# ru1ven/KeypointFusion

Hardware: AMD Instinct MI355X
Metric: RGB-D img/sec fwd (B=64, 256x256) (higher is better)
Workload: dtype f32; 1 GPU; KPFusion-convnext-tiny, depth+RGB UNet backbones forward, B=64/GPU 256x256 f32 (BASELINE configs[1]); batch_per_gpu=64, global_batch=64, input=256x256, parallelism=dp1 (batch shards, no collective)

## Files before the change

include/kpf.h:

```cpp
#ifndef KPF_H
#define KPF_H

#ifdef __cplusplus
extern "C" {
#endif

#define KPF_OK 0
#define KPF_EINVAL (-1)
#define KPF_ELAUNCH (-2)

#define KPF_DT_F32 0
#define KPF_DT_BF16 1
#define KPF_DT_F16 2
#define KPF_DT_F32_MMA_BF16 8
#define KPF_DT_F32_MMA_F16 9

#define KPF_ACT_RELU 1u
#define KPF_ACT_GELU 2u
#define KPF_RES_ADD 4u
#define KPF_RES_GAMMA 8u
#define KPF_RELU_AFTER_RES 16u
#define KPF_ACT_LEAKY 64u
#define KPF_IN_SPLIT 128u
#define KPF_W_SPLIT 512u
#define KPF_OUT_SPLIT 256u
#define KPF_OUT_NCHW 32u
#define KPF_ACT_GELU_SAVE 2048u
#define KPF_MMA_BF16 8192u
#define KPF_MMA_F16 16384u
#define KPF_PRO_LN 4096u
#define KPF_RES_GELU_GRAD 1024u

typedef struct kpf_conv_desc {
  int B, IH, IW, Cin;
  int in_ld, in_coff;
  int OH, OW, N;
  int KH, KW, sh, sw, ph, pw;
  int Kp;
  int out_ld, out_coff;
  int res_ld, res_coff;
  unsigned flags;
  float w_unscale;
  int tile_cfg;
  int groups;
  long w_gstride;
} kpf_conv_desc;

int kpf_conv2d_f32(const kpf_conv_desc* d, const float* in, const float* w, const float* bias,
                   const float* pro_scale, const float* pro_shift, const float* gamma, const float* res,
                   float* out, void* stream);

int kpf_dwconv7_ln_f32(const float* x, const float* w_dw, const float* b_dw, const float* ln_w, const float* ln_b,
                       float* y, int B, int H, int W, int C, float eps, void* stream);

int kpf_convnext_mlp_f32(const float* y, const float* x, const float* w1, const float* b1, const float* w2, const float* b2,
                         const float* gamma, float* out, long M, int C, void* stream);
int kpf_convnext_mlp_supported(int C);
int kpf_convnext_mlp_split_f32(const float* y_split, const float* x, const float* w1_split, const float* b1, float w1_unscale,
                               const float* w2_split_perm, const float* b2, float w2_unscale, const float* gamma, float* out, long M,
                               int C, void* stream);
int kpf_convnext_mlp_split_supported(int C);
int kpf_convnext_mlp_h16(const void* y, const void* x, const void* w1, const float* b1, const void* w2_chunks, const float* b2,
                         const float* gamma, void* out, long M, int C, int dtype, void* stream);
int kpf_convnext_mlp_h16_supported(int C);

int kpf_dwconv7_stats_h16(const void* x, const float* w_dw, const float* b_dw, void* y, float* stats, int B, int H, int W, int C, int dtype,
                          void* stream);
int kpf_dwconv7_stats_supported(int H, int W, int C);
long kpf_dwconv7_stats_floats(int B, int H, int W, int C);
int kpf_ln_apply_stats_h16(void* y, const float* stats, const float* ln_w, const float* ln_b, long rows, int C, float eps, int dtype, void* stream);
int kpf_ln_stats_merge(const float* stats, float* mean_rstd, long rows, int C, float eps, void* stream);

int kpf_layernorm_f32(const float* x, const float* w, const float* b, float* y, long rows, int C, float eps, void* stream);

int kpf_dwconv7_ln_split_f32(const float* x, const float* w_dw, const float* b_dw, const float* ln_w, const float* ln_b, float* y,
                             int B, int H, int W, int C, float eps, void* stream);
int kpf_layernorm_split_f32(const float* x, const float* w, const float* b, float* y, long rows, int C, float eps, void* stream);

int kpf_upsample2x_f32(const float* src, float* dst, int B, int H, int W, int C, int dst_ld, int dst_coff, void* stream);

int kpf_nchw_to_nhwc_f32(const float* src, float* dst, int B, int C, int H, int W, int Cpad, void* stream);

int kpf_nhwc_to_nchw_f32(const float* src, float* dst, int B, int C, int H, int W, int src_ld, int src_coff, void* stream);
// ... 321 lines not shown
```

keypointfusion_amd/csrc/kpf_conv.hip:

```cpp
#include "kpf_common.h"
#include <stdlib.h>
#include <type_traits>

namespace {

struct ConvArgs {
  const float* in;
  const float* w;
  const float* bias;
  const float* ps;
  const float* pt;
  const float* gamma;
  const float* res;
  float* out;
  int M, N, K, Kp;
  int IH, IW, Cin, in_ld, in_coff;
  int OH, OW, ohow, KH, KW, sh, sw, ph, pw;
  int out_ld, out_coff, res_ld, res_coff;
  const float* zero;
  float w_unscale;
  unsigned flags;
  int tilesN, nblk;
  int vec;
  int dbg;
// ... 29 lines not shown
__device__ __forceinline__ float gelu_h16(float x) { return kpf_gelu_h16(x); }
enum { ARITH_F32 = 0, ARITH_SPLIT = 1, ARITH_SPLIT_W = 2, ARITH_BF16 = 3, ARITH_F16 = 4, ARITH_R_BF16 = 5, ARITH_R_F16 = 6 };
template <int ARITH>
__device__ __forceinline__ float gelu_of(float x) {
  if constexpr (ARITH == ARITH_BF16 || ARITH == ARITH_F16) return gelu_h16(x);
  else return gelu_erf(x);
}

enum { EPI_LIN = 0, EPI_GELU = 1, EPI_RES = 2, EPI_GGRAD = 3, EPI_GELU2 = 4 };
__device__ __forceinline__ float gelu_exact_erf(float v) { return 0.5f * v * (1.0f + erff(v * 0.70710678118654752440f)); }
__device__ __forceinline__ float gelu_grad_erf(float v) {
  const float cdf = 0.5f * (1.0f + erff(v * 0.70710678118654752440f));
  return cdf + v * 0.3989422804014327f * __expf(-0.5f * v * v);
}
#ifndef STORE4
#define STORE4(p, v) *reinterpret_cast<f32x4*>(p) = (v)
#endif

typedef __attribute__((address_space(3))) void lds_void_t;
typedef __attribute__((address_space(1))) void gbl_void_t;

__device__ __attribute__((aligned(16))) float kpf_zero16[4] = {0.f, 0.f, 0.f, 0.f};

#ifdef KPF_DBG_TIME
__device__ unsigned long long kpf_dbg_t[8 * 8192];
#define KPF_STAMP(i) do { if (threadIdx.x == 0 && blockIdx.x < 8192) { kpf_dbg_t[8 * blockIdx.x + (i)] = __builtin_readcyclecounter(); \
    if ((i) == 0) { kpf_dbg_t[8 * blockIdx.x + 4] = __builtin_amdgcn_s_memrealtime(); kpf_dbg_t[8 * blockIdx.x + 6] = __builtin_amdgcn_s_getreg((4 << 0) | (0 << 6) | (31 << 11)) | ((unsigned long long)__builtin_amdgcn_s_getreg((20 << 0) | (0 << 6) | (3 << 11)) << 32); } \
    if ((i) == 3) kpf_dbg_t[8 * blockIdx.x + 5] = __builtin_amdgcn_s_memrealtime(); } } while (0)
#else
#define KPF_STAMP(i)
#endif
constexpr int BK = 32;

template <int TM, int TN, int WM, int WN, bool IS1X1, bool HAS_PRO, int EPI, int ARITH, int NS>
__device__ __forceinline__ void igemm_body(const ConvArgs& a) {
  constexpr bool SPLIT = ARITH == ARITH_SPLIT || ARITH == ARITH_SPLIT_W;
  constexpr bool H16 = ARITH == ARITH_BF16 || ARITH == ARITH_F16;
  using TH = typename std::conditional<ARITH == ARITH_BF16, bf16_t, f16_t>::type;
  constexpr int BM = 16 * TM * WM;
  constexpr int BN = 16 * TN * WN;
  constexpr int NW = WM * WN;
  constexpr int RPP = 8 * NW;
  constexpr int AP = (BM + RPP - 1) / RPP;
  constexpr int BP = (BN + RPP - 1) / RPP;
  constexpr bool R16 = ARITH == ARITH_R_BF16 || ARITH == ARITH_R_F16;
  constexpr bool WHOLE = NS > 2 || ARITH == ARITH_F32 || R16;
  constexpr int BMR = WHOLE ? AP * RPP : BM;
  constexpr int BNR = WHOLE ? BP * RPP : BN;
  constexpr int TILE = (BMR + BNR) * BK;
  constexpr int CNT = AP + BP;
  static_assert(NW == 4 || NW == 8, "4 or 8 waves per workgroup");
  static_assert(NS >= 1 && (NS < 2 || (NS - 2) * CNT < 64), "vmcnt is a 6-bit counter");
  static_assert(BM % 8 == 0 && BN % 8 == 0, "tile granularity");

  extern __shared__ __attribute__((aligned(16))) float lds[];

  const int tid = threadIdx.x;
  const int lane = tid & 63;
  const int wave = __builtin_amdgcn_readfirstlane(tid >> 6);
  const int wm = wave % WM, wn = wave / WM;
  KPF_STAMP(0);
  if constexpr (ARITH == ARITH_F32 && NS == 2) {
    if (a.skew > 0 && (int)blockIdx.x < 512 && blockIdx.y == 0) {
      const unsigned tg = __builtin_amdgcn_s_getreg(4 | (16 << 6) | (3 << 11));
      if (tg & 1)
        for (int i = 0; i < a.skew; ++i) __builtin_amdgcn_s_sleep(32);
    }
  }
// ... 111 lines not shown
    }
  }
  if (NS <= 2) __syncthreads();

  KPF_STAMP(1);
  if constexpr (ARITH == ARITH_F32 && NS == 2) {
    auto read_frags = [&](int buf, int s16, f32x4(&xf)[TM], f32x4(&wf)[TN]) {
      const float* xrow = lds + buf * TILE + (wm * TM * 16 + fr) * BK;
      const float* wrow = lds + buf * TILE + BMR * BK + (wn * TN * 16 + fr) * BK;
      const int sc = (((4 * s16 + fg) ^ rsw) << 2);
#pragma unroll
      for (int j = 0; j < TM; ++j) xf[j] = *reinterpret_cast<const f32x4*>(xrow + j * 16 * BK + sc);
#pragma unroll
      for (int i = 0; i < TN; ++i) wf[i] = *reinterpret_cast<const f32x4*>(wrow + i * 16 * BK + sc);
    };
    auto prologue = [&](int kt, int s16, f32x4(&xf)[TM]) {
      if constexpr (HAS_PRO) {
        const int kk = kt * BK + 16 * s16 + 4 * fg;
        const f32x4 sp = *reinterpret_cast<const f32x4*>(pro_s + kk);
        const f32x4 tp = *reinterpret_cast<const f32x4*>(pro_t + kk);
#pragma unroll
        for (int j = 0; j < TM; ++j)
#pragma unroll
          for (int e = 0; e < 4; ++e) xf[j][e] = fmaxf(fmaf(xf[j][e], sp[e], tp[e]), 0.f);
      }
    };
    auto mma = [&](int e, const f32x4(&xf)[TM], const f32x4(&wf)[TN]) {
#pragma unroll
      for (int i = 0; i < TN; ++i)
#pragma unroll
        for (int j = 0; j < TM; ++j) acc[i][j] = __builtin_amdgcn_mfma_f32_16x16x4f32(wf[i][e], xf[j][e], acc[i][j], 0, 0, 0);
    };
    f32x4 xa[TM], wa[TN], xb[TM], wb[TN];
    read_frags(0, 0, xa, wa);
    if (nk > 1) stage(1, 1);
    for (int kt = 0; kt + 1 < nk; ++kt) {
      const int cur = kt & 1;
      read_frags(cur, 1, xb, wb);
      prologue(kt, 0, xa);
#pragma unroll
      for (int e = 0; e < 4; ++e) mma(e, xa, wa);
      prologue(kt, 1, xb);
#pragma unroll
      for (int e = 0; e < 3; ++e) mma(e, xb, wb);
      __builtin_amdgcn_sched_barrier(0);
      asm volatile("s_waitcnt vmcnt(0) lgkmcnt(0)" ::: "memory");
      __builtin_amdgcn_s_barrier();
      __builtin_amdgcn_sched_barrier(0);
      read_frags(cur ^ 1, 0, xa, wa);
      stage(kt + 2 < nk ? kt + 2 : nk - 1, cur);
      mma(3, xb, wb);
      __builtin_amdgcn_sched_group_barrier(0x100, TM + TN, 0);
#pragma unroll
      for (int q = 0; q < AP + BP; ++q) {
        __builtin_amdgcn_sched_group_barrier(0x008, (TM * TN) / (AP + BP) > 0 ? (TM * TN) / (AP + BP) : 1, 0);
        __builtin_amdgcn_sched_group_barrier(0x020, 1, 0);
      }
    }
    {
      const int kt = nk - 1, cur = kt & 1;
      read_frags(cur, 1, xb, wb);
      prologue(kt, 0, xa);
#pragma unroll
      for (int e = 0; e < 4; ++e) mma(e, xa, wa);
      prologue(kt, 1, xb);
#pragma unroll
// ... 1089 lines not shown
    }
  }
  static const bool no_kxk = getenv("KPF_NO_KXK16") != nullptr;
  if (!no_kxk && !pointwise && !pro_scale && a.groups <= 1 && !(fl & (KPF_RES_GELU_GRAD | KPF_ACT_GELU_SAVE | KPF_OUT_NCHW)) && a.M >= 16384) {
    const long tm256 = ((long)a.M + 255) / 256;
    if (a.N % 256 == 0 && tm256 * (a.N / 256) >= 256) best = 26;
    else if (a.N % 128 == 0 && tm256 * (a.N / 128) >= 256) best = 8;
    else if (a.N == 64) best = 2;
  }
  static const int forced = []() { const char* e = getenv("KPF_FORCE_CFG16"); return e ? atoi(e) : -1; }();
  if (forced >= 0 && (forced != 30 || ok8)) best = forced;
  if (d->tile_cfg > 0 && (d->tile_cfg != 31 || ok8)) best = d->tile_cfg - 1;
  if (best == 30) return dtype == KPF_DT_BF16 ? launch_8ph<ARITH_BF16>(a, st) : launch_8ph<ARITH_F16>(a, st);
#ifdef KPF_FAST_BUILD
  return launch_cfg_h16<4, 4, 2, 2, 2>(a, fast1x1, pointwise, dtype, st);
#endif
  switch (best) {
    case 0: return occ ? launch_cfg_h16<4, 4, 2, 2, 1>(a, fast1x1, pointwise, dtype, st) : launch_cfg_h16<4, 4, 2, 2, 2>(a, fast1x1, pointwise, dtype, st);
    case 1: return launch_cfg_h16<4, 3, 2, 2, 2>(a, fast1x1, pointwise, dtype, st);
    case 2: return launch_cfg_h16<2, 4, 4, 1, 2>(a, fast1x1, pointwise, dtype, st);
    case 5: return launch_cfg_h16<2, 4, 2, 2, 2>(a, fast1x1, pointwise, dtype, st);
    case 6: return occ ? launch_cfg_h16<2, 2, 2, 2, 1>(a, fast1x1, pointwise, dtype, st) : launch_cfg_h16<2, 2, 2, 2, 2>(a, fast1x1, pointwise, dtype, st);
    case 8: return launch_cfg_h16<4, 4, 4, 2, 2>(a, fast1x1, pointwise, dtype, st);
    case 20: return launch_cfg_h16<4, 4, 4, 2, 3>(a, fast1x1, pointwise, dtype, st);
    case 21: return launch_cfg_h16<4, 4, 2, 2, 3>(a, fast1x1, pointwise, dtype, st);
    case 22: return launch_cfg_h16<4, 4, 2, 2, 4>(a, fast1x1, pointwise, dtype, st);
    case 26: return launch_cfg_h16<8, 4, 2, 4, 2>(a, fast1x1, pointwise, dtype, st);
    case 41: return launch_cfg_h16<2, 2, 2, 2, 4>(a, fast1x1, pointwise, dtype, st);
    case 44: return launch_cfg_h16<2, 1, 1, 4, 8>(a, fast1x1, pointwise, dtype, st);
    default: return launch_cfg_h16<2, 1, 1, 4, 2>(a, fast1x1, pointwise, dtype, st);
  }
}
#else
extern "C" int kpf_conv2d_f32(const kpf_conv_desc* d, const float* in, const float* w, const float* bias,
                              const float* pro_scale, const float* pro_shift, const float* gamma, const float* res,
                              float* out, void* stream) {
  KPF_REQUIRE(d && in && w && out, "kpf_conv2d_f32: null pointer");
  KPF_REQUIRE(d->B > 0 && d->OH > 0 && d->OW > 0 && d->N > 0 && d->Cin > 0, "kpf_conv2d_f32: empty shape");
  KPF_REQUIRE(d->Cin % 4 == 0 && d->in_ld % 4 == 0 && d->in_coff % 4 == 0,
              "kpf_conv2d_f32: Cin/in_ld/in_coff must be multiples of 4 (got %d/%d/%d)", d->Cin, d->in_ld, d->in_coff);
  KPF_REQUIRE(d->Kp % 32 == 0 && d->Kp >= d->KH * d->KW * d->Cin, "kpf_conv2d_f32: Kp=%d must be a multiple of 32 and >= K=%d",
              d->Kp, d->KH * d->KW * d->Cin);
  KPF_REQUIRE(kpf_aligned16(in) && kpf_aligned16(w) && kpf_aligned16(out), "kpf_conv2d_f32: pointers must be 16-byte aligned");
  const unsigned fl = d->flags;
  if (!(fl & KPF_OUT_NCHW))
    KPF_REQUIRE(d->out_coff >= 0 && d->out_coff + d->N <= d->out_ld, "kpf_conv2d_f32: bad output slice ld=%d coff=%d N=%d",
                d->out_ld, d->out_coff, d->N);
  if (fl & KPF_RES_ADD)
    KPF_REQUIRE(res && kpf_aligned16(res) && d->res_coff >= 0 && d->res_coff + d->N <= d->res_ld, "kpf_conv2d_f32: bad residual");
  if (fl & KPF_RES_GAMMA) KPF_REQUIRE(gamma && (fl & KPF_RES_ADD), "kpf_conv2d_f32: RES_GAMMA needs gamma and RES_ADD");
  KPF_REQUIRE((pro_scale == nullptr) == (pro_shift == nullptr), "kpf_conv2d_f32: prologue needs both scale and shift");
  KPF_REQUIRE(((fl & KPF_ACT_RELU) != 0) + ((fl & KPF_ACT_GELU) != 0) + ((fl & KPF_ACT_LEAKY) != 0) <= 1, "kpf_conv2d_f32: one activation only");
  KPF_REQUIRE(!((fl & KPF_RES_ADD) && (fl & (KPF_ACT_RELU | KPF_ACT_GELU | KPF_ACT_LEAKY))), "kpf_conv2d_f32: activation before a residual add is not supported");
  KPF_REQUIRE(!((fl & KPF_ACT_LEAKY) && pro_scale), "kpf_conv2d_f32: LeakyReLU is not combined with an operand prologue");
  KPF_REQUIRE(!(fl & KPF_RELU_AFTER_RES) || (fl & KPF_RES_ADD), "kpf_conv2d_f32: RELU_AFTER_RES needs RES_ADD");
  KPF_REQUIRE(!(fl & KPF_RES_GELU_GRAD) || ((fl & KPF_RES_ADD) && !(fl & (KPF_RES_GAMMA | KPF_RELU_AFTER_RES | KPF_OUT_NCHW))), "kpf_conv2d_f32: RES_GELU_GRAD goes with RES_ADD alone");
  KPF_REQUIRE(!(fl & KPF_ACT_GELU_SAVE) || ((fl & KPF_ACT_GELU) && !(fl & (KPF_RES_ADD | KPF_OUT_NCHW)) && res && kpf_aligned16(res) && d->res_coff >= 0 && d->res_coff + d->N <= d->res_ld),
              "kpf_conv2d_f32: ACT_GELU_SAVE goes with ACT_GELU and a second output buffer in the res slot (res_ld / res_coff describe it)");
  KPF_REQUIRE((long)d->B * d->OH * d->OW < (1l << 31) && (long)d->B * d->IH * d->IW < (1l << 31), "kpf_conv2d_f32: too many pixels");

  ConvArgs a;
  a.in = in; a.w = w; a.bias = bias; a.ps = pro_scale; a.pt = pro_shift; a.gamma = gamma; a.res = res; a.out = out;
  a.M = d->B * d->OH * d->OW; a.N = d->N; a.K = d->KH * d->KW * d->Cin; a.Kp = d->Kp;
  a.IH = d->IH; a.IW = d->IW; a.Cin = d->Cin; a.in_ld = d->in_ld; a.in_coff = d->in_coff;
  a.OH = d->OH; a.OW = d->OW; a.ohow = d->OH * d->OW; a.KH = d->KH; a.KW = d->KW;
  a.sh = d->sh; a.sw = d->sw; a.ph = d->ph; a.pw = d->pw;
  a.out_ld = d->out_ld; a.out_coff = d->out_coff; a.res_ld = d->res_ld; a.res_coff = d->res_coff;
  {
    static const float* zero_of_dev[64] = {nullptr};
    int dev = 0;
    if (hipGetDevice(&dev) != hipSuccess || dev < 0 || dev >= 64) dev = 0;
    if (!zero_of_dev[dev]) {
      void* p = nullptr;
      if (hipGetSymbolAddress(&p, HIP_SYMBOL(kpf_zero16)) != hipSuccess || !p) {
        kpf_set_error("kpf_conv2d_f32: cannot resolve the zero page");
        return KPF_ELAUNCH;
      }
      zero_of_dev[dev] = static_cast<const float*>(p);
    }
    a.zero = zero_of_dev[dev];
  }
  a.flags = fl; a.tilesN = 0; a.nblk = 0; a.dbg = 0; a.skew = 0; a.st_policy = 0;
  {
    static const int st_mb = []() { const char* e = getenv("KPF_F32_ST_MB"); return e ? atoi(e) : 0; }();
    if (st_mb > 0 && (long)d->B * d->OH * d->OW * d->N * 4 >= (long)st_mb * 1000000) a.st_policy = 2;
  }
  a.w_unscale = (fl & (KPF_IN_SPLIT | KPF_W_SPLIT)) ? d->w_unscale : 1.0f;
  if (fl & (KPF_IN_SPLIT | KPF_W_SPLIT))
    KPF_REQUIRE(d->w_unscale > 0.f && d->Cin % 32 == 0 && d->in_coff % 4 == 0, "kpf_conv2d_f32: split operands need w_unscale > 0 and Cin %% 32 == 0 (Cin=%d)", d->Cin);
  if (fl & KPF_IN_SPLIT) KPF_REQUIRE(d->in_coff % 32 == 0 && d->in_ld % 32 == 0 && !pro_scale, "kpf_conv2d_f32: split activations need in_ld, in_coff multiples of 32 and no operand prologue");
  if (fl & KPF_OUT_SPLIT)
    KPF_REQUIRE(d->N % 32 == 0 && d->out_coff % 32 == 0 && d->out_ld % 32 == 0 && !(fl & KPF_OUT_NCHW),
                "kpf_conv2d_f32: split output needs N, out_ld, out_coff multiples of 32 (N=%d ld=%d coff=%d)", d->N, d->out_ld, d->out_coff);
  a.vec = (d->out_ld % 4 == 0 && d->out_coff % 4 == 0 && (!(fl & KPF_RES_ADD) || (d->res_ld % 4 == 0 && d->res_coff % 4 == 0))) ? 1 : 0;
  a.groups = d->groups > 1 ? d->groups : 1; a.g_in = a.g_out = 0; a.g_w = 0;
  if (a.groups > 1) {
    KPF_REQUIRE(!(fl & (KPF_RES_GAMMA | KPF_OUT_NCHW | KPF_IN_SPLIT | KPF_W_SPLIT | KPF_OUT_SPLIT)) && !pro_scale && d->w_gstride % 4 == 0,
                "kpf_conv2d_f32: a grouped launch takes no layer scale / prologue / NCHW output / split operands, and needs w_gstride %% 4 == 0");
    KPF_REQUIRE(d->in_coff + d->groups * d->Cin <= d->in_ld && d->out_coff + d->groups * d->N <= d->out_ld, "kpf_conv2d_f32: the groups' channel slices exceed the pixel stride");
    KPF_REQUIRE(!(fl & (KPF_RES_ADD | KPF_ACT_GELU_SAVE)) || d->res_coff + d->groups * d->N <= d->res_ld,
                "kpf_conv2d_f32: the groups' residual / saved pre-activation slices exceed the pixel stride");
    a.g_in = d->Cin; a.g_out = d->N; a.g_w = d->w_gstride;
    if ((d->out_coff + d->N) % 4 || ((fl & KPF_RES_ADD) && (d->res_coff + d->N) % 4)) a.vec = 0;
  }
  const bool is1x1 = d->KH == 1 && d->KW == 1 && d->sh == 1 && d->sw == 1 && d->ph == 0 && d->pw == 0 &&
                     d->IH == d->OH && d->IW == d->OW && d->Cin % 32 == 0 && d->Kp == d->Cin;
  hipStream_t st = reinterpret_cast<hipStream_t>(stream);

  int best = 0;
  double bc = 1e30;
  static const int forced = []() { const char* e = getenv("KPF_FORCE_CFG"); return e ? atoi(e) : -1; }();
  for (int i = 0; i < (int)(sizeof(kCfgs) / sizeof(kCfgs[0])); ++i) {
    const double c = cfg_cost(kCfgs[i], a.M, a.N, a.groups);
// ... 64 lines not shown
```

keypointfusion_amd/engine.py:

```python
import ctypes as C
import math

import torch

from . import lib as L
from .spec import CONVNEXT, parse_net

BN_EPS = 1e-5
FORCE_UNFUSED_MLP = bool(int(__import__("os").environ.get("KPF_UNFUSED_MLP", "0")))
GEMM_MODE = __import__("os").environ.get("KPF_GEMM", "f32")
assert GEMM_MODE in ("split", "f32"), "KPF_GEMM must be 'split' or 'f32'"
F16_MAX = 65504.0
AUTOTUNE = bool(int(__import__("os").environ.get("KPF_AUTOTUNE", "0")))
_TILE_RULES = {tuple(int(v) for v in r.split("=")[0].split(":")): int(r.split("=")[1]) + 1 for r in __import__("os").environ.get("KPF_TILE_RULES", "").split(",") if r}


PROFILE = None
FORCE_TILE = 0


def _launch(kernel, flops, nbytes, shape, fn):
    if PROFILE is None:
        return fn()
    e0, e1 = torch.cuda.Event(enable_timing=True), torch.cuda.Event(enable_timing=True)
    e0.record()
    r = fn()
    e1.record()
    PROFILE.append((kernel, e0, e1, flops, nbytes, shape))
    return r


def _ptr(t):
    return C.c_void_p(t.data_ptr()) if t is not None else C.c_void_p(0)


def _stream():
    return C.c_void_p(torch.cuda.current_stream().cuda_stream)


class Act:
    __slots__ = ("buf", "B", "H", "W", "C", "ld", "coff", "split")

    def __init__(self, buf, B, H, W, C, ld=None, coff=0, split=False):
        self.buf, self.B, self.H, self.W, self.C = buf, B, H, W, C
        self.ld = C if ld is None else ld
# ... 135 lines not shown
    w = pc.w
    if x.split:
        flags |= L.KPF_IN_SPLIT
        w, d.w_unscale = pc.split_weights()
    elif GEMM_MODE == "split" and pc.Cin % 32 == 0 and pc.split_allowed:
        flags |= L.KPF_W_SPLIT
        w, d.w_unscale = pc.split_weights()
    if out_split:
        flags |= L.KPF_OUT_SPLIT
        out.split = True
    elif out is not None and out_nchw is None:
        out.split = False
    d.flags = flags
    d.groups, d.w_gstride = getattr(pc, "groups", 0), getattr(pc, "w_gstride", 0)
    M = B * OH * OW
    if AUTOTUNE:
        key = (M, IH, IW, flags, in_ld, in_coff, d.out_ld, d.out_coff, d.res_ld, d.res_coff)
        cfg = pc.tuned.get(key)
        if cfg is None and PROFILE is None and not torch.cuda.is_current_stream_capturing():
            cfg = pc.tuned[key] = _autotune(lib, d, x, w, pc, gamma, res, optr, flags)
        d.tile_cfg = cfg or 0
    if _TILE_RULES and not AUTOTUNE:
        d.tile_cfg = _TILE_RULES.get((M, pc.N, pc.K, pc.KH), 0)
    if FORCE_TILE:
        d.tile_cfg = FORCE_TILE
    nbytes = 4.0 * (B * IH * IW * pc.Cin + pc.N * pc.K + M * pc.N * (2 if res is not None else 1))
    ng = max(1, d.groups)
    _launch("igemm_split_kernel" if flags & (L.KPF_IN_SPLIT | L.KPF_W_SPLIT) else "igemm_f32_kernel", pc.flops(M) * ng, nbytes * ng, (M, pc.N, pc.K, pc.KH, pc.KW),
            lambda: L.check(lib.kpf_conv2d_f32(C.byref(d), _ptr(x.buf), _ptr(w), _ptr(pc.b), _ptr(pc.ps), _ptr(pc.pt), _ptr(gamma),
                                               _ptr(res.buf if res is not None else None), _ptr(optr), _stream()), "kpf_conv2d_f32"))
    return out


def _autotune(lib, d, x, w, pc, gamma, res, optr, flags):
    ncfg = int(lib.kpf_conv_num_tile_cfgs())
    split = bool(flags & (L.KPF_IN_SPLIT | L.KPF_W_SPLIT))
    cands = [i for i in range(ncfg) if split or i < 9 or i == 17]
    out_t = optr
    if res is not None and res.buf.data_ptr() == optr.data_ptr():
        out_t = torch.empty_like(optr)
    args = (_ptr(x.buf), _ptr(w), _ptr(pc.b), _ptr(pc.ps), _ptr(pc.pt), _ptr(gamma), _ptr(res.buf if res is not None else None), _ptr(out_t), _stream())
    torch.cuda.synchronize()
    best, best_t = 0, float("inf")
    for c in cands:
        d.tile_cfg = c + 1
        if lib.kpf_conv2d_f32(C.byref(d), *args) != 0:
            continue
        e0, e1 = torch.cuda.Event(enable_timing=True), torch.cuda.Event(enable_timing=True)
        e0.record()
        for _ in range(3):
            lib.kpf_conv2d_f32(C.byref(d), *args)
        e1.record()
        e1.synchronize()
        t = e0.elapsed_time(e1)
        if t < best_t:
            best, best_t = c + 1, t
    return best


def layernorm(x, w, b, eps, out=None, out_split=False):
    lib = L.load()
    assert x.ld == x.C and x.coff == 0
    out = x if out is None else out
    fn = lib.kpf_layernorm_split_f32 if out_split else lib.kpf_layernorm_f32
    L.check(fn(_ptr(x.buf), _ptr(w), _ptr(b), _ptr(out.buf), x.B * x.H * x.W, x.C, eps, _stream()), "kpf_layernorm_f32")
    out.split = out_split
# ... 32 lines not shown


def nhwc_to_nchw(x):
    lib = L.load()
    out = torch.empty(x.B, x.C, x.H, x.W, device=x.buf.device, dtype=torch.float32)
    L.check(lib.kpf_nhwc_to_nchw_f32(_ptr(x.buf), _ptr(out), x.B, x.C, x.H, x.W, x.ld, x.coff, _stream()),
            "kpf_nhwc_to_nchw_f32")
    return out


def maxpool3x3s2(x):
    lib = L.load()
    assert x.ld == x.C and x.coff == 0
    OH, OW = (x.H - 1) // 2 + 1, (x.W - 1) // 2 + 1
    out = Act.empty(x.B, OH, OW, x.C, x.buf.device)
    L.check(lib.kpf_maxpool3x3s2_f32(_ptr(x.buf), _ptr(out.buf), x.B, x.H, x.W, x.C, _stream()), "kpf_maxpool3x3s2_f32")
    return out


class ResidualPlan:

    def __init__(self, sd, p, device):
        cin = sd[p + ".conv1.conv.weight"].shape[1]
        cout = sd[p + ".conv3.conv.weight"].shape[0]
        self.cin, self.cout = cin, cout
        self.c1 = PackedConv(sd[p + ".conv1.conv.weight"], sd[p + ".conv1.conv.bias"], device,
                             fold_bn=bn_scale_shift(sd, p + ".bn2"), prologue=bn_scale_shift(sd, p + ".bn1"))
        self.c2 = PackedConv(sd[p + ".conv2.conv.weight"], sd[p + ".conv2.conv.bias"], device, pad=1,
                             fold_bn=bn_scale_shift(sd, p + ".bn3"))
        self.c3 = PackedConv(sd[p + ".conv3.conv.weight"], sd[p + ".conv3.conv.bias"], device)
        self.skip = None
        if cin != cout:
            self.skip = PackedConv(sd[p + ".skip_layer.conv.weight"], sd[p + ".skip_layer.conv.bias"], device)

    def __call__(self, x, out=None):
        h = conv(self.c1, x, flags=L.KPF_ACT_RELU)
        h = conv(self.c2, h, flags=L.KPF_ACT_RELU)
        if out is None:
            out = Act.empty(x.B, x.H, x.W, self.cout, x.buf.device)
        if self.skip is not None:
            conv(self.skip, x, out=out)
            return conv(self.c3, h, out=out, res=out)
        return conv(self.c3, h, out=out, res=x)

    def flops(self, M):
        f = self.c1.flops(M) + self.c2.flops(M) + self.c3.flops(M)
        return f + (self.skip.flops(M) if self.skip else 0)


class ConvNeXtBlockPlan:

    def __init__(self, sd, p, device):
        c = sd[p + ".gamma"].numel()
        self.C = c
        self.wdw = sd[p + ".dwconv.weight"].detach().float().reshape(c, 49).t().contiguous().to(device)
        self.bdw = sd[p + ".dwconv.bias"].detach().float().to(device)
        self.lnw = sd[p + ".norm.weight"].detach().float().to(device)
        self.lnb = sd[p + ".norm.bias"].detach().float().to(device)
        self.pw1 = PackedConv(sd[p + ".pwconv1.weight"], sd[p + ".pwconv1.bias"], device)
        self.pw2 = PackedConv(sd[p + ".pwconv2.weight"], sd[p + ".pwconv2.bias"], device)
        self.gamma = sd[p + ".gamma"].detach().float().to(device)
        ln_bound = math.sqrt(c) * float(self.lnw.abs().max()) + float(self.lnb.abs().max())
        h_bound = self.pw1.row_l1() * ln_bound + float(self.pw1.b.abs().max())
        self.split_ok = c % 32 == 0 and ln_bound < F16_MAX and h_bound < F16_MAX
        self.pw1.split_allowed = self.pw2.split_allowed = self.split_ok
        self.fused_split = GEMM_MODE == "split" and self.split_ok and bool(L.load().kpf_convnext_mlp_split_supported(c))
        if self.fused_split:
            self.w1s, self.us1 = self.pw1.split_weights()
            w2 = self.pw2.w.double().cpu()
            perm = torch.tensor([32 * q + k for q in range(4 * c // 32) for k in MLP_HIDDEN_PERM])
            w2s, self.us2 = split_pack(w2[:, perm])
            self.w2s = w2s.to(device)
        self.fused = bool(L.load().kpf_convnext_mlp_supported(c))
        if self.fused:
            self.w1 = sd[p + ".pwconv1.weight"].detach().float().contiguous().to(device)
            self.b1 = sd[p + ".pwconv1.bias"].detach().float().contiguous().to(device)
# ... 435 lines not shown
```

keypointfusion_amd/lib.py:

```python
import ctypes as C
import os

_HERE = os.path.dirname(os.path.abspath(__file__))
LIB_PATH = os.environ.get("KPF_LIB_PATH") or os.path.join(_HERE, "libkpf_hip.so")

KPF_ACT_RELU = 1
KPF_ACT_GELU = 2
KPF_RES_ADD = 4
KPF_RES_GAMMA = 8
KPF_RELU_AFTER_RES = 16
KPF_RES_GELU_GRAD = 1024
KPF_ACT_GELU_SAVE = 2048
KPF_PRO_LN = 4096
KPF_DT_F32_MMA_BF16, KPF_DT_F32_MMA_F16 = 8, 9
KPF_MMA_BF16, KPF_MMA_F16 = 8192, 16384
KPF_OUT_NCHW = 32
KPF_ACT_LEAKY = 64
KPF_IN_SPLIT = 128
KPF_OUT_SPLIT = 256
KPF_W_SPLIT = 512
KPF_DT_F32, KPF_DT_BF16, KPF_DT_F16 = 0, 1, 2
ABI_VERSION = 18


# ... 33 lines not shown
    "kpf_layernorm_split_f32": [_P, _P, _P, _P, C.c_long, C.c_int, C.c_float, _P],
    "kpf_dwconv7_ln_split_f32": [_P, _P, _P, _P, _P, _P, C.c_int, C.c_int, C.c_int, C.c_int, C.c_float, _P],
    "kpf_upsample2x_f32": [_P, _P, C.c_int, C.c_int, C.c_int, C.c_int, C.c_int, C.c_int, _P],
    "kpf_nchw_to_nhwc_f32": [_P, _P, C.c_int, C.c_int, C.c_int, C.c_int, C.c_int, _P],
    "kpf_nhwc_to_nchw_f32": [_P, _P, C.c_int, C.c_int, C.c_int, C.c_int, C.c_int, C.c_int, _P],
    "kpf_maxpool3x3s2_f32": [_P, _P, C.c_int, C.c_int, C.c_int, C.c_int, _P],
    "kpf_inv3x3_f32": [_P, _P, C.c_int, C.c_int, _P],
    "kpf_offset2joint_f32": [_P] * 8 + [C.c_int, C.c_int, C.c_int, C.c_float, C.c_int, C.c_int, _P],
    "kpf_img2pcl_top4_f32": [_P] * 9 + [C.c_int] * 6 + [_P],
    "kpf_point_assemble_f32": [_P] * 9 + [C.c_int, C.c_int, C.c_int, C.c_float, _P],
    "kpf_softmax_pool_f32": [_P, _P, _P, _P, C.c_int, C.c_int, _P],
    "kpf_ball_group_f32": [_P, _P, _P, _P, C.c_int, _P, _P, C.c_int, C.c_int, C.c_float, C.c_float, C.c_float, _P],
    "kpf_group_max_f32": [_P, _P, C.c_long, C.c_int, C.c_int, C.c_int, C.c_int, _P],
    "kpf_ball_group_stacked_f32": [_P, _P, _P, _P, C.c_int, _P, _P, _P, C.c_int, C.c_int, C.c_float, C.c_float, C.c_float, _P],
    "kpf_ball_group_bwd_f32": [_P, C.c_int, _P, _P, _P, _P, C.c_int, C.c_int, C.c_int, _P],
    "kpf_slices_sum_relu_forward": [_P, _P, C.c_long, C.c_int, C.c_int, C.c_int, _P],
    "kpf_slices_sum_relu_backward": [_P, _P, _P, _P, C.c_long, C.c_int, C.c_int, C.c_int, _P],
    "kpf_group_max_train_forward": [_P, _P, _P, C.c_long, C.c_int, C.c_int, _P],
    "kpf_group_max_train_backward": [_P, C.c_int, _P, _P, C.c_long, C.c_int, C.c_int, _P],
    "kpf_heat_gam_gate_f32": [_P, _P, _P, C.c_int] + [_P] * 10 + [C.c_int] * 4 + [_P],
    "kpf_gate_reduce_f32": [_P, _P, _P, _P, _P, C.c_int, C.c_int, _P],
    "kpf_tr_encoder_f32": [_P, C.c_int, C.c_int, _P, _P, _P, _P, C.c_int, C.c_int, _P],
    "kpf_xattn_layer_f32": [_P, _P, _P, _P, C.c_int, C.c_int, C.c_int, _P],
    "kpf_conv2d_h16": [C.POINTER(ConvDesc), _P, _P, _P, _P, _P, _P, _P, _P, C.c_int, _P],
    "kpf_conv2d_h16_uses_8ph": [C.POINTER(ConvDesc), C.c_int],
    "kpf_conv2d_h16_ln_fold_supported": [C.POINTER(ConvDesc)],
    "kpf_dwconv7_ln_h16": [_P, _P, _P, _P, _P, _P, C.c_int, C.c_int, C.c_int, C.c_int, C.c_float, C.c_int, _P],
    "kpf_layernorm_h16": [_P, C.c_int, _P, _P, _P, C.c_int, C.c_long, C.c_int, C.c_float, _P],
    "kpf_upsample2x_h16": [_P, _P, C.c_int, C.c_int, C.c_int, C.c_int, C.c_int, C.c_int, C.c_int, _P],
    "kpf_cast_h16_f32": [_P, C.c_int, _P, C.c_long, C.c_int, C.c_int, C.c_int, _P],
    "kpf_cast_f32_h16": [_P, _P, C.c_int, C.c_long, _P],
    "kpf_convnext_mlp_f32": [_P] * 8 + [C.c_long, C.c_int, _P],
    "kpf_convnext_mlp_supported": [C.c_int],
    "kpf_convnext_mlp_split_f32": [_P, _P, _P, _P, C.c_float, _P, _P, C.c_float, _P, _P, C.c_long, C.c_int, _P],
    "kpf_convnext_mlp_split_supported": [C.c_int],
    "kpf_convnext_mlp_h16": [_P] * 8 + [C.c_long, C.c_int, C.c_int, _P],
    "kpf_convnext_mlp_h16_supported": [C.c_int],
    "kpf_dwconv7_stats_h16": [_P, _P, _P, _P, _P, C.c_int, C.c_int, C.c_int, C.c_int, C.c_int, _P],
    "kpf_dwconv7_stats_supported": [C.c_int, C.c_int, C.c_int],
    "kpf_ln_apply_stats_h16": [_P, _P, _P, _P, C.c_long, C.c_int, C.c_float, C.c_int, _P],
    "kpf_ln_stats_merge": [_P, _P, C.c_long, C.c_int, C.c_float, _P],
    "kpf_cbam_channel_gate_f32": [_P] * 7 + [C.c_int] * 4 + [_P],
    "kpf_cbam_spatial_gate_f32": [_P, _P, _P, C.c_float, C.c_float, _P, _P, C.c_int, C.c_int, C.c_int, C.c_int, _P],
    "kpf_cbam_apply_f32": [_P] * 5 + [C.c_int] * 3 + [_P],
    "kpf_maxpool2x2_f32": [_P, _P, C.c_int, C.c_int, C.c_int, C.c_int, _P],
    "kpf_upnearest2x_add_f32": [_P, _P, _P, C.c_int, C.c_int, C.c_int, C.c_int, _P],
    "kpf_mano_forward_f32": [_P, C.c_int, _P, C.c_int] + [_P] * 10 + [C.c_int, _P],
    "kpf_tr_encoder_weight_floats": [C.c_int],
    "kpf_conv_num_tile_cfgs": [],
    "kpf_xattn_weight_floats": [],
    "kpf_conv2d_wgrad_f32": [_P] * 5 + [C.c_long] + [C.c_int] * 15 + [_P],
    "kpf_bn_train_forward": [_P, C.c_int, _P, _P, _P, C.c_int, _P, _P, _P, _P, C.c_float, C.c_float, C.c_int, _P, C.c_long, C.c_long, C.c_int, _P],
    "kpf_bn_train_backward": [_P, _P, _P, C.c_int, C.c_int, _P, _P, _P, _P, _P, _P, C.c_int, _P, C.c_long, C.c_long, C.c_int, _P],
    "kpf_bn_train_backward_add": [_P, _P, _P, C.c_int, C.c_int, _P, _P, _P, _P, _P, _P, _P, C.c_int, _P, C.c_long, C.c_long, C.c_int, _P],
    "kpf_bn_train_forward_f32": [_P] * 8 + [C.c_float, C.c_float, C.c_int, _P, C.c_long, C.c_long, C.c_int, _P],
    "kpf_bn_train_backward_f32": [_P] * 9 + [C.c_int, _P, C.c_long, C.c_long, C.c_int, _P],
    "kpf_dwconv7_f32": [_P, _P, _P, _P, C.c_int, C.c_int, C.c_int, C.c_int, _P],
    "kpf_dwconv7_add_f32": [_P, _P, _P, _P, _P, C.c_int, C.c_int, C.c_int, C.c_int, _P],
    "kpf_conv2d_wgrad_h16": [_P, _P, C.c_int] + [_P] * 3 + [C.c_long] + [C.c_int] * 15 + [_P],
    "kpf_conv2d_wgrad_groups": [_P, _P, C.c_int] + [_P] * 3 + [C.c_long] + [C.c_int] * 18 + [_P],
    "kpf_conv2d_wgrad_deferred": [_P, _P, C.c_int] + [_P] * 3 + [C.c_long] + [C.c_int] * 18 + [C.POINTER(WgradReduceDesc), _P],
    "kpf_dwconv7_wgrad_deferred": [_P] * 5 + [C.c_long] + [C.c_int] * 4 + [C.POINTER(WgradReduceDesc), _P],
    "kpf_wgrad_reduce_multi": [C.POINTER(WgradReduceDesc), C.c_int, _P],
    "kpf_row_gather_cols_f32": [_P, C.c_long, C.c_long, C.c_long, _P, _P, _P, C.c_int, C.c_int, C.c_int, C.c_int, C.c_int, _P],
    "kpf_bn_ssr_forward": [_P] * 7 + [C.c_float, C.c_float, _P, C.c_long, C.c_long, C.c_int, C.c_int, C.c_int, _P],
    "kpf_bn_ssr_backward": [_P] * 10 + [C.c_long, C.c_long, C.c_int, C.c_int, C.c_int, _P],
# ... 132 lines not shown
```

Before: 3491 img/s.

## Fuse residual block conv2 3x3 and conv3 1x1 with residual add into one kernel

Adds a kernel that runs the residual block's 3x3 conv2 (bias+ReLU) and keeps its output tile in registers. It then chains the 1x1 conv3 as an extra MFMA stage, with W3 staged through the same LDS buffers, and adds bias and residual in the epilogue. This removes the write and re-read of the mid activation and one launch per block. The cost is more register pressure (a second accumulator array) and a fixed tile config per supported (mid, cout) pair, which bypasses autotuned tiling.

Result: no change. 3523 img/s, median of 6 (+0.9%).

```diff
diff --git a/include/kpf.h b/include/kpf.h
--- a/include/kpf.h
+++ b/include/kpf.h
@@ -49,6 +49,10 @@
 int kpf_conv2d_f32(const kpf_conv_desc* d, const float* in, const float* w, const float* bias,
                    const float* pro_scale, const float* pro_shift, const float* gamma, const float* res,
                    float* out, void* stream);
+
+int kpf_resblock_tail_f32(const kpf_conv_desc* d, const float* in, const float* w2, const float* b2, const float* w3, const float* b3,
+                          int cout, int Kp3, const float* res, float* out, void* stream);
+int kpf_resblock_tail_supported(int mid, int cout);
 
 int kpf_dwconv7_ln_f32(const float* x, const float* w_dw, const float* b_dw, const float* ln_w, const float* ln_b,
                        float* y, int B, int H, int W, int C, float eps, void* stream);
diff --git a/keypointfusion_amd/csrc/kpf_conv.hip b/keypointfusion_amd/csrc/kpf_conv.hip
--- a/keypointfusion_amd/csrc/kpf_conv.hip
+++ b/keypointfusion_amd/csrc/kpf_conv.hip
@@ -85,8 +85,13 @@
 #endif
 constexpr int BK = 32;
 
-template <int TM, int TN, int WM, int WN, bool IS1X1, bool HAS_PRO, int EPI, int ARITH, int NS>
-__device__ __forceinline__ void igemm_body(const ConvArgs& a) {
+struct TailArgs {
+  const float* w3;
+  const float* b3;
+  int Kp3;
+};
+template <int TM, int TN, int WM, int WN, bool IS1X1, bool HAS_PRO, int EPI, int ARITH, int NS, int C3T = 0>
+__device__ __forceinline__ void igemm_body(const ConvArgs& a, const TailArgs& ta = TailArgs{nullptr, nullptr, 0}) {
   constexpr bool SPLIT = ARITH == ARITH_SPLIT || ARITH == ARITH_SPLIT_W;
   constexpr bool H16 = ARITH == ARITH_BF16 || ARITH == ARITH_F16;
   using TH = typename std::conditional<ARITH == ARITH_BF16, bf16_t, f16_t>::type;
@@ -264,6 +269,143 @@
         for (int j = 0; j < TM; ++j) acc[i][j] = __builtin_amdgcn_mfma_f32_16x16x4f32(wf[i][e], xf[j][e], acc[i][j], 0, 0, 0);
     };
     f32x4 xa[TM], wa[TN], xb[TM], wb[TN];
+    if constexpr (C3T > 0) {
+      static_assert(WN == 1 && !IS1X1 && !HAS_PRO && EPI == EPI_LIN, "the chained tail sits on the plain 3x3 convolution of a WN = 1 tile");
+      static_assert((C3T * 16) % RPP == 0 && C3T * 16 <= BMR + BNR, "a W3 K tile is whole staging passes and fits one K buffer");
+      constexpr int C3P = C3T * 16 / RPP;
+      constexpr int KT3 = (TN + 1) / 2;
+      const float* pw3 = ta.w3 + (long)lr * ta.Kp3 + kc;
+      auto stage_w3 = [&](int kt3, int buf) {
+        float* Ws = lds + buf * TILE;
+#pragma unroll
+        for (int p = 0; p < C3P; ++p)
+          __builtin_amdgcn_global_load_lds((gbl_void_t*)(pw3 + (long)p * RPP * ta.Kp3 + kt3 * BK), (lds_void_t*)(Ws + (RPP * p + 8 * wave) * BK), 16, 0, 0);
+      };
+      auto ktile = [&](int kt, auto last) {
+        constexpr bool LAST = decltype(last)::value;
+        const int cur = kt & 1;
+        read_frags(cur, 1, xb, wb);
+#pragma unroll
+        for (int e = 0; e < 4; ++e) mma(e, xa, wa);
+#pragma unroll
+        for (int e = 0; e < 3; ++e) mma(e, xb, wb);
+        __builtin_amdgcn_sched_barrier(0);
+        asm volatile("s_waitcnt vmcnt(0) lgkmcnt(0)" ::: "memory");
+        __builtin_amdgcn_s_barrier();
+        __builtin_amdgcn_sched_barrier(0);
+        read_frags(cur ^ 1, 0, xa, wa);
+        if constexpr (LAST) stage_w3(0, cur);
+        else stage(kt + 2, cur);
+        mma(3, xb, wb);
+        constexpr int ND = LAST ? C3P : AP + BP;
+        __builtin_amdgcn_sched_group_barrier(0x100, TM + TN, 0);
+#pragma unroll
+        for (int q = 0; q < ND; ++q) {
+          __builtin_amdgcn_sched_group_barrier(0x008, (TM * TN) / ND > 0 ? (TM * TN) / ND : 1, 0);
+          __builtin_amdgcn_sched_group_barrier(0x020, 1, 0);
+        }
+      };
+      read_frags(0, 0, xa, wa);
+      stage(1, 1);
+      for (int kt = 0; kt + 2 < nk; ++kt) ktile(kt, std::false_type{});
+      ktile(nk - 2, std::true_type{});
+      {
+        const int cur = (nk - 1) & 1;
+        read_frags(cur, 1, xb, wb);
+#pragma unroll
+        for (int e = 0; e < 4; ++e) mma(e, xa, wa);
+#pragma unroll
+        for (int e = 0; e < 4; ++e) mma(e, xb, wb);
+      }
+#pragma unroll
+      for (int i = 0; i < TN; ++i) {
+        const f32x4 bv = a.bias ? *reinterpret_cast<const f32x4*>(a.bias + i * 16 + fg * 4) : zero4;
+#pragma unroll
+        for (int j = 0; j < TM; ++j)
+#pragma unroll
+          for (int e = 0; e < 4; ++e) acc[i][j][e] = fmaxf(acc[i][j][e] + bv[e], 0.f);
+      }
+      f32x4 acc3[C3T][TM];
+#pragma unroll
+      for (int i = 0; i < C3T; ++i)
+#pragma unroll
+        for (int j = 0; j < TM; ++j) acc3[i][j] = zero4;
+#pragma unroll
+      for (int t3 = 0; t3 < KT3; ++t3) {
+        const int b3 = (nk + t3) & 1;
+        __builtin_amdgcn_sched_barrier(0);
+        asm volatile("s_waitcnt vmcnt(0) lgkmcnt(0)" ::: "memory");
+        __builtin_amdgcn_s_barrier();
+        __builtin_amdgcn_sched_barrier(0);
+        if (t3 + 1 < KT3) stage_w3(t3 + 1, b3 ^ 1);
+#pragma unroll
+        for (int s16 = 0; s16 < 2; ++s16) {
+          const int tn = 2 * t3 + s16;
+          if (tn < TN) {
+            const float* wrow = lds + b3 * TILE + fr * BK + (((4 * s16 + fg) ^ rsw) << 2);
+            constexpr int CH = C3T > 8 ? C3T / 2 : C3T;
+#pragma unroll
+            for (int c = 0; c < C3T; c += CH) {
+              f32x4 w3f[CH];
+#pragma unroll
+              for (int i = 0; i < CH; ++i) w3f[i] = *reinterpret_cast<const f32x4*>(wrow + (c + i) * 16 * BK);
+#pragma unroll
+              for (int e = 0; e < 4; ++e)
+#pragma unroll
+                for (int i = 0; i < CH; ++i)
+#pragma unroll
+                  for (int j = 0; j < TM; ++j)
+                    acc3[c + i][j] = __builtin_amdgcn_mfma_f32_16x16x4f32(w3f[i][e], acc[tn < TN ? tn : 0][j][e], acc3[c + i][j], 0, 0, 0);
+            }
+          }
+        }
+      }
+      KPF_STAMP(2);
+#pragma unroll
+      for (int i = 0; i < C3T; ++i) {
+        const f32x4 bv = *reinterpret_cast<const f32x4*>(ta.b3 + i * 16 + fg * 4);
+#pragma unroll
+        for (int j = 0; j < TM; ++j)
+#pragma unroll
+          for (int e = 0; e < 4; ++e) acc3[i][j][e] = acc3[i][j][e] + bv[e];
+      }
+      if (m0 + BM <= a.M && a.vec) {
+        f32x4 rv[2][C3T];
+        auto load_res = [&](int j, f32x4(&r)[C3T]) {
+          const long m = m0 + (wm * TM + j) * 16 + fr;
+#pragma unroll
+          for (int i = 0; i < C3T; ++i) r[i] = *reinterpret_cast<const f32x4*>(a.res + m * a.res_ld + a.res_coff + i * 16 + fg * 4);
+        };
+        load_res(0, rv[0]);
+#pragma unroll
+        for (int j = 0; j < TM; ++j) {
+          if (j + 1 < TM) load_res(j + 1, rv[(j + 1) & 1]);
+          const long m = m0 + (wm * TM + j) * 16 + fr;
+#pragma unroll
+          for (int i = 0; i < C3T; ++i) {
+            f32x4 v = acc3[i][j];
+#pragma unroll
+            for (int e = 0; e < 4; ++e) v[e] += rv[j & 1][i][e];
+            STORE4(a.out + m * a.out_ld + a.out_coff + i * 16 + fg * 4, v);
+          }
+        }
+      } else {
+#pragma unroll
+        for (int j = 0; j < TM; ++j) {
+          const long m = m0 + (wm * TM + j) * 16 + fr;
+          if (m >= a.M) continue;
+#pragma unroll
+          for (int i = 0; i < C3T; ++i)
+#pragma unroll
+            for (int e = 0; e < 4; ++e) {
+              const int n = i * 16 + fg * 4 + e;
+              a.out[m * a.out_ld + a.out_coff + n] = acc3[i][j][e] + a.res[m * a.res_ld + a.res_coff + n];
+            }
+        }
+      }
+      KPF_STAMP(3);
+      return;
+    }
     read_frags(0, 0, xa, wa);
     if (nk > 1) stage(1, 1);
     for (int kt = 0; kt + 1 < nk; ++kt) {
@@ -1419,6 +1561,81 @@
   }
 }
 #else
+static const float* kpf_zero_page() {
+  static const float* zero_of_dev[64] = {nullptr};
+  int dev = 0;
+  if (hipGetDevice(&dev) != hipSuccess || dev < 0 || dev >= 64) dev = 0;
+  if (!zero_of_dev[dev]) {
+    void* p = nullptr;
+    if (hipGetSymbolAddress(&p, HIP_SYMBOL(kpf_zero16)) != hipSuccess || !p) return nullptr;
+    zero_of_dev[dev] = static_cast<const float*>(p);
+  }
+  return zero_of_dev[dev];
+}
+
+template <int TM, int TN, int WM, int C3T>
+__global__ __launch_bounds__(64 * WM, 2) void resblock_tail_f32_kernel(const ConvArgs a, const TailArgs ta) {
+  igemm_body<TM, TN, WM, 1, false, false, EPI_LIN, ARITH_F32, 2, C3T>(a, ta);
+}
+
+template <int TM, int TN, int WM, int C3T>
+int launch_tail(ConvArgs& a, const TailArgs& ta, hipStream_t st) {
+  constexpr int BM = 16 * TM * WM, BN = 16 * TN, RPP = 8 * WM;
+  constexpr int BMR = (BM + RPP - 1) / RPP * RPP, BNR = (BN + RPP - 1) / RPP * RPP;
+  const size_t lds = (size_t)2 * (BMR + BNR) * BK * sizeof(float);
+  a.tilesN = 1;
+  a.nblk = (a.M + BM - 1) / BM;
+  void (*kern)(const ConvArgs, const TailArgs) = resblock_tail_f32_kernel<TM, TN, WM, C3T>;
+  static std::atomic<bool> lds_opt_in[KPF_MAX_DEVICES];
+  if (!kpf_raise_lds_limit(reinterpret_cast<const void*>(kern), lds_opt_in)) {
+    kpf_set_error("kpf_resblock_tail_f32: cannot raise the dynamic LDS limit");
+    return KPF_ELAUNCH;
+  }
+  hipLaunchKernelGGL(kern, dim3(a.nblk), dim3(64 * WM), lds, st, a, ta);
+  return kpf_check_launch("kpf_resblock_tail_f32");
+}
+
+extern "C" int kpf_resblock_tail_supported(int mid, int cout) {
+  return (mid == 64 && cout == 128) || (mid == 48 && cout == 96) || (mid == 96 && cout == 192);
+}
+
+extern "C" int kpf_resblock_tail_f32(const kpf_conv_desc* d, const float* in, const float* w2, const float* b2, const float* w3,
+                                     const float* b3, int cout, int Kp3, const float* res, float* out, void* stream) {
+  KPF_REQUIRE(d && in && w2 && b2 && w3 && b3 && res && out, "kpf_resblock_tail_f32: null pointer");
+  KPF_REQUIRE(d->B > 0 && d->OH > 0 && d->OW > 0, "kpf_resblock_tail_f32: empty shape");
+  KPF_REQUIRE(kpf_resblock_tail_supported(d->N, cout), "kpf_resblock_tail_f32: unsupported block (mid=%d, cout=%d): see kpf_resblock_tail_supported", d->N, cout);
+  KPF_REQUIRE(d->Cin == d->N && d->KH == 3 && d->KW == 3 && d->sh == 1 && d->sw == 1 && d->ph == 1 && d->pw == 1 && d->IH == d->OH && d->IW == d->OW,
+              "kpf_resblock_tail_f32: conv2 must be a 3x3 / stride 1 / pad 1 convolution mid -> mid");
+  KPF_REQUIRE(d->in_ld % 4 == 0 && d->in_coff % 4 == 0 && d->in_coff >= 0 && d->in_coff + d->Cin <= d->in_ld, "kpf_resblock_tail_f32: bad input slice ld=%d coff=%d", d->in_ld, d->in_coff);
+  KPF_REQUIRE(d->Kp % 32 == 0 && d->Kp >= 9 * d->Cin && d->Kp >= 64, "kpf_resblock_tail_f32: Kp=%d must be a multiple of 32 and >= 9 * mid", d->Kp);
+  KPF_REQUIRE(Kp3 == (d->N + 31) / 32 * 32, "kpf_resblock_tail_f32: Kp3=%d must be mid rounded up to 32", Kp3);
+  KPF_REQUIRE(d->flags == KPF_ACT_RELU && d->groups <= 1, "kpf_resblock_tail_f32: flags must be KPF_ACT_RELU (conv2's activation), one group");
+  KPF_REQUIRE(d->out_coff >= 0 && d->out_coff + cout <= d->out_ld && d->res_coff >= 0 && d->res_coff + cout <= d->res_ld,
+              "kpf_resblock_tail_f32: bad output / residual slice (out ld=%d coff=%d, res ld=%d coff=%d, cout=%d)", d->out_ld, d->out_coff, d->res_ld, d->res_coff, cout);
+  KPF_REQUIRE(kpf_aligned16(in) && kpf_aligned16(w2) && kpf_aligned16(b2) && kpf_aligned16(w3) && kpf_aligned16(b3) && kpf_aligned16(res) && kpf_aligned16(out),
+              "kpf_resblock_tail_f32: pointers must be 16-byte aligned");
+  KPF_REQUIRE((long)d->B * d->OH * d->OW < (1l << 31), "kpf_resblock_tail_f32: too many pixels");
+  ConvArgs a;
+  a.in = in; a.w = w2; a.bias = b2; a.ps = a.pt = a.gamma = nullptr; a.res = res; a.out = out;
+  a.M = d->B * d->OH * d->OW; a.N = d->N; a.K = 9 * d->Cin; a.Kp = d->Kp;
+  a.IH = d->IH; a.IW = d->IW; a.Cin = d->Cin; a.in_ld = d->in_ld; a.in_coff = d->in_coff;
+  a.OH = d->OH; a.OW = d->OW; a.ohow = d->OH * d->OW; a.KH = 3; a.KW = 3; a.sh = a.sw = 1; a.ph = a.pw = 1;
+  a.out_ld = d->out_ld; a.out_coff = d->out_coff; a.res_ld = d->res_ld; a.res_coff = d->res_coff;
+  a.zero = kpf_zero_page();
+  if (!a.zero) {
+    kpf_set_error("kpf_resblock_tail_f32: cannot resolve the zero page");
+    return KPF_ELAUNCH;
+  }
+  a.w_unscale = 1.0f; a.flags = d->flags; a.tilesN = 1; a.nblk = 0; a.dbg = 0; a.st_policy = 0; a.skew = 0;
+  a.vec = (d->out_ld % 4 == 0 && d->out_coff % 4 == 0 && d->res_ld % 4 == 0 && d->res_coff % 4 == 0) ? 1 : 0;
+  a.groups = 1; a.g_in = a.g_out = 0; a.g_w = 0;
+  const TailArgs ta{w3, b3, Kp3};
+  hipStream_t st = reinterpret_cast<hipStream_t>(stream);
+  if (d->N == 64) return launch_tail<2, 4, 4, 8>(a, ta, st);
+  if (d->N == 48) return launch_tail<4, 3, 4, 6>(a, ta, st);
+  return launch_tail<2, 6, 4, 12>(a, ta, st);
+}
+
 extern "C" int kpf_conv2d_f32(const kpf_conv_desc* d, const float* in, const float* w, const float* bias,
                               const float* pro_scale, const float* pro_shift, const float* gamma, const float* res,
                               float* out, void* stream) {
@@ -1453,19 +1670,10 @@
   a.OH = d->OH; a.OW = d->OW; a.ohow = d->OH * d->OW; a.KH = d->KH; a.KW = d->KW;
   a.sh = d->sh; a.sw = d->sw; a.ph = d->ph; a.pw = d->pw;
   a.out_ld = d->out_ld; a.out_coff = d->out_coff; a.res_ld = d->res_ld; a.res_coff = d->res_coff;
-  {
-    static const float* zero_of_dev[64] = {nullptr};
-    int dev = 0;
-    if (hipGetDevice(&dev) != hipSuccess || dev < 0 || dev >= 64) dev = 0;
-    if (!zero_of_dev[dev]) {
-      void* p = nullptr;
-      if (hipGetSymbolAddress(&p, HIP_SYMBOL(kpf_zero16)) != hipSuccess || !p) {
-        kpf_set_error("kpf_conv2d_f32: cannot resolve the zero page");
-        return KPF_ELAUNCH;
-      }
-      zero_of_dev[dev] = static_cast<const float*>(p);
-    }
-    a.zero = zero_of_dev[dev];
+  a.zero = kpf_zero_page();
+  if (!a.zero) {
+    kpf_set_error("kpf_conv2d_f32: cannot resolve the zero page");
+    return KPF_ELAUNCH;
   }
   a.flags = fl; a.tilesN = 0; a.nblk = 0; a.dbg = 0; a.skew = 0; a.st_policy = 0;
   {
diff --git a/keypointfusion_amd/engine.py b/keypointfusion_amd/engine.py
--- a/keypointfusion_amd/engine.py
+++ b/keypointfusion_amd/engine.py
@@ -11,6 +11,8 @@
 GEMM_MODE = __import__("os").environ.get("KPF_GEMM", "f32")
 assert GEMM_MODE in ("split", "f32"), "KPF_GEMM must be 'split' or 'f32'"
 F16_MAX = 65504.0
+FORCE_UNFUSED_RESBLOCK = bool(int(__import__("os").environ.get("KPF_UNFUSED_RESBLOCK", "0")))
+_TAIL_MIDS = tuple(int(v) for v in __import__("os").environ.get("KPF_RESBLOCK_TAIL_MID", "").split(",") if v)
 AUTOTUNE = bool(int(__import__("os").environ.get("KPF_AUTOTUNE", "0")))
 _TILE_RULES = {tuple(int(v) for v in r.split("=")[0].split(":")): int(r.split("=")[1]) + 1 for r in __import__("os").environ.get("KPF_TILE_RULES", "").split(",") if r}
 
@@ -212,6 +214,25 @@
     return out
 
 
+def resblock_tail(c2, c3, h, out, res):
+    lib = L.load()
+    assert h.C == c2.Cin == c2.N == c3.Cin and c3.Kp == (c2.N + 31) // 32 * 32 and not h.split
+    assert (out.B, out.H, out.W, out.C) == (h.B, h.H, h.W, c3.N) and (res.B, res.H, res.W, res.C) == (h.B, h.H, h.W, c3.N)
+    d = L.ConvDesc()
+    d.B, d.IH, d.IW, d.Cin, d.in_ld, d.in_coff = h.B, h.H, h.W, c2.Cin, h.ld, h.coff
+    d.OH, d.OW, d.N = h.H, h.W, c2.N
+    d.KH, d.KW, d.sh, d.sw, d.ph, d.pw, d.Kp = c2.KH, c2.KW, c2.sh, c2.sw, c2.ph, c2.pw, c2.Kp
+    d.out_ld, d.out_coff, d.res_ld, d.res_coff = out.ld, out.coff, res.ld, res.coff
+    d.flags = L.KPF_ACT_RELU
+    M = h.B * h.H * h.W
+    nbytes = 4.0 * (M * c2.Cin + c2.N * c2.K + c3.N * c3.K + 2 * M * c3.N)
+    _launch("resblock_tail_f32_kernel", c2.flops(M) + c3.flops(M), nbytes, (M, c3.N, c2.K, c2.KH, c2.KW),
+            lambda: L.check(lib.kpf_resblock_tail_f32(C.byref(d), _ptr(h.buf), _ptr(c2.w), _ptr(c2.b), _ptr(c3.w), _ptr(c3.b), c3.N, c3.Kp,
+                                                      _ptr(res.buf), _ptr(out.buf), _stream()), "kpf_resblock_tail_f32"))
+    out.split = False
+    return out
+
+
 def _autotune(lib, d, x, w, pc, gamma, res, optr, flags):
     ncfg = int(lib.kpf_conv_num_tile_cfgs())
     split = bool(flags & (L.KPF_IN_SPLIT | L.KPF_W_SPLIT))
@@ -310,16 +331,21 @@
         self.skip = None
         if cin != cout:
             self.skip = PackedConv(sd[p + ".skip_layer.conv.weight"], sd[p + ".skip_layer.conv.bias"], device)
+        self.fused_tail = bool(L.load().kpf_resblock_tail_supported(self.c2.N, cout)) and (not _TAIL_MIDS or self.c2.N in _TAIL_MIDS)
 
     def __call__(self, x, out=None):
         h = conv(self.c1, x, flags=L.KPF_ACT_RELU)
-        h = conv(self.c2, h, flags=L.KPF_ACT_RELU)
         if out is None:
             out = Act.empty(x.B, x.H, x.W, self.cout, x.buf.device)
+        res = x if self.skip is None else out
+        if self.fused_tail and not FORCE_UNFUSED_RESBLOCK and not (AUTOTUNE or _TILE_RULES or FORCE_TILE):
+            if self.skip is not None:
+                conv(self.skip, x, out=out)
+            return resblock_tail(self.c2, self.c3, h, out, res)
+        h = conv(self.c2, h, flags=L.KPF_ACT_RELU)
         if self.skip is not None:
             conv(self.skip, x, out=out)
-            return conv(self.c3, h, out=out, res=out)
-        return conv(self.c3, h, out=out, res=x)
+        return conv(self.c3, h, out=out, res=res)
 
     def flops(self, M):
         f = self.c1.flops(M) + self.c2.flops(M) + self.c3.flops(M)
diff --git a/keypointfusion_amd/lib.py b/keypointfusion_amd/lib.py
--- a/keypointfusion_amd/lib.py
+++ b/keypointfusion_amd/lib.py
@@ -89,6 +89,8 @@
     "kpf_cast_f32_h16": [_P, _P, C.c_int, C.c_long, _P],
     "kpf_convnext_mlp_f32": [_P] * 8 + [C.c_long, C.c_int, _P],
     "kpf_convnext_mlp_supported": [C.c_int],
+    "kpf_resblock_tail_f32": [C.POINTER(ConvDesc), _P, _P, _P, _P, _P, C.c_int, C.c_int, _P, _P, _P],
+    "kpf_resblock_tail_supported": [C.c_int, C.c_int],
     "kpf_convnext_mlp_split_f32": [_P, _P, _P, _P, C.c_float, _P, _P, C.c_float, _P, _P, C.c_long, C.c_int, _P],
     "kpf_convnext_mlp_split_supported": [C.c_int],
     "kpf_convnext_mlp_h16": [_P] * 8 + [C.c_long, C.c_int, C.c_int, _P],
```
